# oneam/h264bsd

Hardware: AMD Instinct MI355X
Metric: 1080p macroblocks/s (higher is better)
Workload: dtype u8; 1 GPU; 256 concurrent copies of test_1920x1080.h264 per GPU (73 pictures x 8160 MB), kernel-only replay from HBM-resident frame jobs, inter+intra reconstruction + in-loop deblocking; streams_per_gpu=256, parallelism=streams/1, stream_groups=1, row_bands=library default (engine.hip TailConfig)

## Files before the change

### h264bsd_amd/capi.py

```python
import ctypes
import os
import subprocess

import numpy as np

HERE = os.path.dirname(os.path.abspath(__file__))
CSRC = os.path.join(HERE, "csrc")
LIB_PATH = os.path.join(HERE, "lib", "libh264bsd_mi355x.so")
BENCH_LIB_PATH = os.path.join(HERE, "lib", "libh264bsd_mi355x_bench.so")
if os.environ.get("H264BSD_VARIANT"):
    BENCH_LIB_PATH = os.path.join(HERE, "lib_" + os.environ["H264BSD_VARIANT"], "libh264bsd_mi355x_bench.so")

(H264BSD_RDY, H264BSD_PIC_RDY, H264BSD_HDRS_RDY, H264BSD_ERROR, H264BSD_PARAM_SET_ERROR,
 H264BSD_MEMALLOC_ERROR) = range(6)

EXPORTED_SYMBOLS = [
    "h264bsdInit", "h264bsdDecode", "h264bsdShutdown", "h264bsdNextOutputPicture",
    "h264bsdNextOutputPictureRGBA", "h264bsdNextOutputPictureBGRA", "h264bsdNextOutputPictureYCbCrA",
    "h264bsdPicWidth", "h264bsdPicHeight", "h264bsdVideoRange", "h264bsdMatrixCoefficients",
    "h264bsdCroppingParams", "h264bsdSampleAspectRatio", "h264bsdCheckValidParamSets", "h264bsdFlushBuffer",
    "h264bsdProfile", "h264bsdAlloc", "h264bsdFree", "h264bsdConvertToRGBA", "h264bsdConvertToBGRA",
    "h264bsdConvertToYCbCrA",
    "h264bsdmiInitCapture", "h264bsdmiNextOutputInfo", "h264bsdmiNextOutputPictureDevice", "h264bsdmiNextOutputTensorBatch", "h264bsdmiNextOutputTensorBatchColour", "h264bsdmiNextOutputTensorBatchResize", "h264bsdmiOutputTensorRegions", "h264bsdmiOutputTensorRemap", "h264bsdmiSetMotionExport", "h264bsdmiOutputMotionRegions", "h264bsdmiOutputRegionStats", "h264bsdmiKeepCurrentPictures", "h264bsdmiOutputRegionChange", "h264bsdmiOutputRegionShift", "h264bsdmiOutputCellMaps", "h264bsdmiOutputCellBoxes", "h264bsdmiJobFinalize", "h264bsdmiDeviceCount", "h264bsdmiSetDevice", "h264bsdmiFlush", "h264bsdmiFlushAsync", "h264bsdmiDeviceErrors",
    "h264bsdmiDecodePicture", "h264bsdmiDecodePictureBatch", "h264bsdmiNextOutputPictureBatch", "h264bsdmiPullAndDecodePictureBatch", "h264bsdmiSetParserThreads", "h264bsdmiSetInputReadOnly", "h264bsdmiSetCopyElision",
    "h264bsdmiReplayCreate", "h264bsdmiReplayCreateStaggered", "h264bsdmiReplayCreateDesync", "h264bsdmiReplayCreateSched", "h264bsdmiReplayReschedule", "h264bsdmiReplayDestroy", "h264bsdmiReplayRun", "h264bsdmiReplaySync",
    "h264bsdmiReplayFetch", "h264bsdmiReplayChecksums", "h264bsdmiReplayConvert", "h264bsdmiReplayFetchConverted",
    "h264bsdmiReplayTimings", "h264bsdmiReplaySetConvert", "h264bsdmiReplayConvertTimings", "h264bsdmiReplaySetStages", "h264bsdmiReplaySetTimedKernels", "h264bsdmiReplaySetGroups", "h264bsdmiDebugTailProfile", "h264bsdmiDebugSetTail", "h264bsdmiDebugDeviceErrorEvents", "h264bsdmiReplayJobBytes", "h264bsdmiReplayFrameBytes",
]

class DevicePicture(ctypes.Structure):
    _fields_ = [("data", ctypes.c_void_p), ("width", ctypes.c_uint32), ("height", ctypes.c_uint32), ("pitch", ctypes.c_uint32),
                ("format", ctypes.c_uint32), ("picId", ctypes.c_uint32), ("isIdrPic", ctypes.c_uint32),
                ("numErrMbs", ctypes.c_uint32), ("stream", ctypes.c_void_p)]


FMT_RGBA, FMT_BGRA, FMT_YCBCRA, FMT_I420 = 0, 1, 2, 3


class TensorSpec(ctypes.Structure):
    _fields_ = [("data", ctypes.c_void_p), ("width", ctypes.c_uint32), ("height", ctypes.c_uint32), ("layout", ctypes.c_uint32),
                ("dtype", ctypes.c_uint32), ("channels", ctypes.c_uint32), ("crop", ctypes.c_uint32), ("resize", ctypes.c_uint32),
                ("mean", ctypes.c_float * 3), ("std", ctypes.c_float * 3)]


class ColourSpec(ctypes.Structure):
    _fields_ = [("matrix", ctypes.c_uint32), ("range", ctypes.c_uint32), ("chroma", ctypes.c_uint32), ("unspecified", ctypes.c_uint32)]


class ResizeSpec(ctypes.Structure):
    _fields_ = [("filter", ctypes.c_uint32), ("fit", ctypes.c_uint32), ("pad", ctypes.c_float * 3)]


class Region(ctypes.Structure):
    _fields_ = [("instance", ctypes.c_uint32), ("x", ctypes.c_int), ("y", ctypes.c_int), ("w", ctypes.c_uint32), ("h", ctypes.c_uint32)]


class Remap(ctypes.Structure):
    _fields_ = [("instance", ctypes.c_uint32), ("map", ctypes.c_void_p)]

# ... 175 lines not shown
                                          P32, P32, P32, P32, P32]
    L.h264bsdmiOutputCellMaps.restype = ctypes.c_int
    L.h264bsdmiOutputCellBoxes.argtypes = [u32, ctypes.POINTER(vp), u32, ctypes.POINTER(Region), ctypes.POINTER(CellsSpec), ctypes.POINTER(BoxesSpec), vp,
                                           P32, P32, P32, P32, P32]
    L.h264bsdmiOutputCellBoxes.restype = ctypes.c_int
    L.h264bsdmiDecodePicture.argtypes = [vp, u8p, u32, u32, P32, P32]
    L.h264bsdmiDecodePicture.restype = u32
    L.h264bsdmiDecodePictureBatch.argtypes = [u32, ctypes.POINTER(vp), ctypes.POINTER(vp), P32, P32, P32, P32, P32]
    L.h264bsdmiPullAndDecodePictureBatch.argtypes = [u32, ctypes.POINTER(vp), ctypes.POINTER(vp), P32, P32, P32, ctypes.POINTER(vp), P32, P32, P32, P32, P32]
    L.h264bsdmiSetParserThreads.argtypes = [ctypes.c_int]
    L.h264bsdmiSetInputReadOnly.argtypes = [vp, u32]
    L.h264bsdmiSetCopyElision.argtypes = [vp, u32]
    L.h264bsdmiSetCopyElision.restype = ctypes.c_int
    L.h264bsdmiSetDevice.argtypes = [ctypes.c_int]
    L.h264bsdmiDeviceErrors.restype = ctypes.c_uint
    L.h264bsdmiNextOutputPictureBatch.argtypes = [u32, ctypes.POINTER(vp), ctypes.POINTER(vp), P32, P32, P32]
    if not harness:
        return L
    L.h264bsdmiJobFinalize.argtypes = [ctypes.c_void_p, u32, u32]
    L.h264bsdmiReplayCreate.argtypes = [ctypes.POINTER(ctypes.c_void_p), P32, u32, u32]
    L.h264bsdmiReplayCreate.restype = vp
    L.h264bsdmiReplayCreateStaggered.argtypes = [ctypes.POINTER(ctypes.c_void_p), P32, u32, u32, u32]
    L.h264bsdmiReplayCreateStaggered.restype = vp
    L.h264bsdmiReplayCreateDesync.argtypes = [ctypes.POINTER(ctypes.c_void_p), P32, u32, u32, P32, u32, u32]
    L.h264bsdmiReplayCreateDesync.restype = vp
    L.h264bsdmiReplayCreateSched.argtypes = [ctypes.POINTER(ctypes.c_void_p), P32, u32, u32, P32, u32, u32, u32]
    L.h264bsdmiReplayCreateSched.restype = vp
    L.h264bsdmiReplayReschedule.argtypes = [vp, P32, u32, u32, u32]
    L.h264bsdmiReplayDestroy.argtypes = [vp]
    L.h264bsdmiReplayDestroy.restype = None
    L.h264bsdmiReplayRun.argtypes = [vp, u32, u32]
    L.h264bsdmiReplaySync.argtypes = [vp]
    L.h264bsdmiReplayFetch.argtypes = [vp, u32, u32, vp]
    L.h264bsdmiReplayChecksums.argtypes = [vp, u32, vp]
    L.h264bsdmiReplayConvert.argtypes = [vp, u32, ctypes.c_int]
    L.h264bsdmiReplayFetchConverted.argtypes = [vp, u32, vp]
    L.h264bsdmiReplayTimings.argtypes = [vp, ctypes.POINTER(ctypes.c_float), P32]
    L.h264bsdmiReplaySetConvert.argtypes = [vp, ctypes.c_int]
    L.h264bsdmiReplayConvertTimings.argtypes = [vp, ctypes.POINTER(ctypes.c_float), P32]
    L.h264bsdmiReplaySetStages.argtypes = [vp, ctypes.c_uint]
    L.h264bsdmiReplaySetTimedKernels.argtypes = [vp, ctypes.c_uint]
    L.h264bsdmiReplaySetGroups.argtypes = [vp, u32]
    L.h264bsdmiDebugSetTail.argtypes = [u32] * 7
    L.h264bsdmiReplayJobBytes.argtypes = [vp]
    L.h264bsdmiReplayJobBytes.restype = ctypes.c_ulonglong
    L.h264bsdmiReplayFrameBytes.argtypes = [vp]
    L.h264bsdmiReplayFrameBytes.restype = u32
    return L


def device_count():
    return int(api_lib().h264bsdmiDeviceCount())


KEEP = 0xFFFFFFFF


def set_tail(dbk_rows_light=KEEP, dbk_rows_heavy=KEEP, dbk_waves=KEEP, intra_rows_light=KEEP, intra_rows_heavy=KEEP, intra_waves=KEEP,
             band_budget=KEEP):
    lib().h264bsdmiDebugSetTail(dbk_rows_light, dbk_rows_heavy, dbk_waves, intra_rows_light, intra_rows_heavy, intra_waves, band_budget)


def device_errors():
    return int(api_lib().h264bsdmiDeviceErrors())


# ... 798 lines not shown
        self.job_bytes = int(L.h264bsdmiReplayJobBytes(self._h))

    def reschedule(self, odd_offset=0, offsets=None, heavy_lanes=0, heavy_delay=4, groups=1):
        if offsets is None:
            offsets = [odd_offset if s & 1 else 0 for s in range(self.n_streams)]
        self.odd_offset = odd_offset
        self.offsets = [int(o) for o in offsets]
        offs = (ctypes.c_uint32 * self.n_streams)(*self.offsets)
        if self._L.h264bsdmiReplayReschedule(self._h, offs, heavy_lanes, heavy_delay, groups) != 0:
            raise RuntimeError("h264bsdmiReplayReschedule failed")

    def close(self):
        if self._h:
            self._L.h264bsdmiReplayDestroy(self._h)
            self._h = None

    __del__ = close

    def run(self, first=0, count=None):
        count = self.n_pics - first if count is None else count
        if self._L.h264bsdmiReplayRun(self._h, first, count) != 0:
            raise RuntimeError("h264bsdmiReplayRun failed")

    def sync(self):
        if self._L.h264bsdmiReplaySync(self._h) != 0:
            raise RuntimeError("h264bsdmiReplaySync failed")

    def fetch(self, stream, slot):
        out = np.empty(self.frame_bytes, dtype=np.uint8)
        if self._L.h264bsdmiReplayFetch(self._h, stream, slot, out.ctypes.data) != 0:
            raise RuntimeError("h264bsdmiReplayFetch failed")
        return out

    def checksums(self, slot):
        out = np.empty(self.n_streams, dtype=np.uint64)
        if self._L.h264bsdmiReplayChecksums(self._h, slot, out.ctypes.data) != 0:
            raise RuntimeError("h264bsdmiReplayChecksums failed")
        return out

    def set_convert(self, fmt, trailing=True, hosting=True, conv_waves=0):
        if fmt >= 0:
            fmt |= (0 if trailing else 0x100) | (0 if hosting else 0x200) | ((conv_waves & 15) << 16)
        if self._L.h264bsdmiReplaySetConvert(self._h, fmt) != 0:
            raise RuntimeError("h264bsdmiReplaySetConvert failed")

    def convert_timings(self):
        ms, n = ctypes.c_float(0), ctypes.c_uint32(0)
        if self._L.h264bsdmiReplayConvertTimings(self._h, ctypes.byref(ms), ctypes.byref(n)) != 0:
            raise RuntimeError("h264bsdmiReplayConvertTimings failed")
        return ms.value, n.value

    def convert(self, slot, fmt):
        if self._L.h264bsdmiReplayConvert(self._h, slot, fmt) != 0:
            raise RuntimeError("h264bsdmiReplayConvert failed")

    def fetch_converted(self, stream, n_pixels):
        out = np.empty(n_pixels, dtype=np.uint32)
        if self._L.h264bsdmiReplayFetchConverted(self._h, stream, out.ctypes.data) != 0:
            raise RuntimeError("h264bsdmiReplayFetchConverted failed")
        return out

    def set_groups(self, n):
        if self._L.h264bsdmiReplaySetGroups(self._h, n) != 0:
            raise RuntimeError('h264bsdmiReplaySetGroups failed')

    def set_stages(self, mask):
# ... 18 lines not shown
```

### h264bsd_amd/csrc/engine.hip

```cpp
#include <hip/hip_runtime.h>
#include <stdio.h>
#include <stdlib.h>
#include <string.h>
#include <deque>
#include <memory>
#include <mutex>
#include <vector>
#include <algorithm>
#include "kernels.hip.h"
#include "kernels/k_tensor_out.hip.h"
#include "kernels/k_tensor_aa.hip.h"
#include "kernels/k_tensor_roi.hip.h"
#include "kernels/k_tensor_remap.hip.h"
#include "kernels/k_motion.hip.h"
#include "kernels/k_region_stats.hip.h"
#include "kernels/k_keep.hip.h"
#include "kernels/k_region_change.hip.h"
#include "kernels/k_region_shift.hip.h"
#include "kernels/k_cell_maps.hip.h"
#include "kernels/k_cell_boxes.hip.h"
#include "engine.h"
#include "hip_owned.h"
#include "tick_plan.h"
#include "../../include/h264bsd_mi355x_bench.h"
// ... 301 lines not shown
        const bool heavy = h->n_intra * 4u > h->n_mbs;
        d.heavy = heavy ? 1 : 0;
        d.dbk_bands = bands_for(h->height_mbs, heavy ? tc.dbk_rows_heavy : tc.dbk_rows_light);
        d.intra_bands = h->intra_down_deps ? 1 : bands_for(h->height_mbs, heavy ? tc.intra_rows_heavy : tc.intra_rows_light);
    }
    d.err = dev_err;
    d.conv_src = nullptr; d.conv_dst = nullptr; d.conv_fmt = 0; d.conv_pad = 0;
    for (uint32_t k = 0; k < FJ_MAX_SLOTS; k++) d.slot[k] = k < h->n_slots ? dev_frames + (size_t)k * frame_bytes : nullptr;
    if (shape) {
        shape->n_frames++;
        shape->max_mbs = std::max(shape->max_mbs, h->n_mbs);
        shape->max_copy = std::max(shape->max_copy, h->n_copy);
        shape->max_gen = std::max(shape->max_gen, h->n_gen);
        shape->max_gen_uni = std::max(shape->max_gen_uni, h->n_gen_uniform);
        shape->max_gen_quad = std::max(shape->max_gen_quad, h->n_gen_quad);
        shape->max_gen_rest = std::max(shape->max_gen_rest, h->n_gen - h->n_gen_uniform - h->n_gen_quad);
        shape->max_dbk = std::max(shape->max_dbk, h->n_dbk);
        shape->any_deblock |= h->any_deblock != 0;
        shape->max_levels = std::max(shape->max_levels, h->n_intra_levels);
        shape->max_w = std::max<uint32_t>(shape->max_w, h->width_mbs);
        shape->max_h = std::max<uint32_t>(shape->max_h, h->height_mbs);
        shape->any_tail |= h->n_intra_levels != 0 || h->any_deblock != 0;
        shape->n_heavy += d.heavy;
        if (h->any_deblock) (d.heavy ? shape->want_heavy : shape->want_light)[0] = std::max<uint32_t>((d.heavy ? shape->want_heavy : shape->want_light)[0], d.dbk_bands);
        if (h->n_intra_levels) (d.heavy ? shape->want_heavy : shape->want_light)[1] = std::max<uint32_t>((d.heavy ? shape->want_heavy : shape->want_light)[1], d.intra_bands);
        if (h->n_intra_levels && h->intra_down_deps) shape->intra_whole = true;
    }
}

struct TickTimers { Event ev[6]; Event sev[5]; bool on = false; bool copy_timed = false; unsigned mask = 31u; };

static void launch_kdbk(hipStream_t st, const FrameDesc *d_desc, const TickShape &s, uint32_t launches[5])
{
    hipLaunchKernelGGL(h264k::k_dbk, dim3(std::min<uint32_t>((s.max_dbk + 4 * DBK_WG_WAVES - 1) / (4 * DBK_WG_WAVES), DBK_WGS * 4 / DBK_WG_WAVES), s.n_frames), dim3(64 * DBK_WG_WAVES), 0, st, d_desc);
    if (launches) launches[2]++;
}
template <int PATH> static void launch_inter(hipStream_t st, const FrameDesc *d_desc, uint32_t n_max, uint32_t n_frames)
{
    constexpr uint32_t per_wg = INTER_WG_WAVES * h264k::inter_per_wave<PATH>();
    if (n_max) hipLaunchKernelGGL(h264k::k_recon_inter<PATH>, dim3((n_max + per_wg - 1) / per_wg, n_frames), dim3(64 * INTER_WG_WAVES), 0, st, d_desc);
}
std::mutex g_tail_lds_mu;
size_t g_tail_lds[2][2][MAX_DEVICES] = {};
static int tail_prepare(hipStream_t st, int which, const BandPlan &bp, const void *fn, uint32_t **tickets)
{
    const bool banded = bp.bands > 1;
    *tickets = banded ? tickets_for(st) : nullptr;
    if (banded && !*tickets) return -1;
    int dev = 0;
    HIP_TRY(hipGetDevice(&dev));
    std::lock_guard<std::mutex> lk(g_tail_lds_mu);
    if (bp.lds > g_tail_lds[which][banded][dev]) {
        HIP_TRY(hipFuncSetAttribute(fn, hipFuncAttributeMaxDynamicSharedMemorySize, (int)bp.lds));
        g_tail_lds[which][banded][dev] = bp.lds;
    }
    return 0;
}

int launch_tick(hipStream_t st, const FrameDesc *d_desc, const TickShape &s, TickTimers *tt, uint32_t launches[5],
                unsigned stages = 7u, const SideLane *side = nullptr, unsigned long long *prof = nullptr)
{
    const bool timed = tt && tt->on;
    const unsigned tmask = timed ? tt->mask : 0u;
    auto boundary = [&](unsigned i) -> int {
        if ((((tmask << 1) | tmask) >> i) & 1u) HIP_TRY(hipEventRecord(tt->ev[i], st));
        return 0;
    };
// ... 1344 lines not shown
```

### h264bsd_amd/csrc/kernels/k_dbk.hip.h

```cpp
#pragma once
namespace h264k {
#ifndef DBK_WGS
#define DBK_WGS 32
#endif
#ifndef DBK_WG_WAVES
#define DBK_WG_WAVES 4
#endif
__global__ __launch_bounds__(64 * DBK_WG_WAVES) void k_dbk(const FrameDesc *__restrict__ frames)
{
    __shared__ uint32_t s_tab[32 + 64];
    if (threadIdx.x < 64) {
        const uint32_t t = threadIdx.x, ok = t < 52;
        reinterpret_cast<uint8_t *>(s_tab)[t] = ok ? c_alpha[t] : 0;
        reinterpret_cast<uint8_t *>(s_tab)[64 + t] = ok ? c_beta[t] : 0;
        s_tab[32 + t] = ok ? (uint32_t)c_tc0[t][0] | ((uint32_t)c_tc0[t][1] << 8) | ((uint32_t)c_tc0[t][2] << 16) : 0u;
    }
    __syncthreads();
    const FrameDesc &fd = FD_REF(frames, blockIdx.y);
    const int m = threadIdx.x & 15;
    const int wmb = fd.wmb;
    const uint32_t n_dbk = fd.n_dbk;
    uint32_t di = blockIdx.x * (4 * DBK_WG_WAVES) + (threadIdx.x >> 4);
    const bool live0 = di < n_dbk;
    if (__ballot(live0) == 0ull) return;
    uint32_t mb = live0 ? fd.dbki[di] : 0u;
    bool live = live0;
  for (;;) {
    const uint32_t ndi = di + (4u * DBK_WG_WAVES) * gridDim.x;
    uint32_t nmb = mb;
    const bool nlive = live && ndi < n_dbk;
    if (nlive) nmb = fd.dbki[ndi];
    const uint32_t mbx = mb - mb_row(fd, mb) * (uint32_t)wmb;
    const uint32_t mbl = mbx ? mb - 1 : mb, mbt = mb >= (uint32_t)wmb ? mb - wmb : mb;
    FjMbRec q, pl, pt;
    const int dir = m >> 3, e = (m >> 1) & 3, kh = m & 1;
    int qx[2], qy[2], px[2], py[2];
    uint32_t mva[2], mvb[2];
#pragma unroll
    for (int kk = 0; kk < 2; kk++) {
        const int k = 2 * kh + kk;
        qx[kk] = dir ? k : e; qy[kk] = dir ? e : k;
        px[kk] = dir ? k : (e ? e - 1 : 3); py[kk] = dir ? (e ? e - 1 : 3) : k;
    }
    {
        const H264K_GLOBAL uint8_t *rq = (const H264K_GLOBAL uint8_t *)(fd.recs + mb), *rl = (const H264K_GLOBAL uint8_t *)(fd.recs + mbl),
                                   *rt = (const H264K_GLOBAL uint8_t *)(fd.recs + mbt);
        uint4 w[6] = { ld16g(rq), ld16g(rq + 16), ld16g(rl), ld16g(rl + 16), ld16g(rt), ld16g(rt + 16) };
#pragma unroll
        for (int i = 0; i < 6; i++) asm volatile("" : "+v"(w[i].x), "+v"(w[i].y), "+v"(w[i].z), "+v"(w[i].w));
        __builtin_memcpy(&q, &w[0], 32); __builtin_memcpy(&pl, &w[2], 32); __builtin_memcpy(&pt, &w[4], 32);
    }
    {
        const FjMbRec &pr = e ? q : (dir ? pt : pl);
        const bool q_one = (q.pred & FJ_PRED_UNIFORM_MV) || q.kind != FJ_MB_INTER, p_one = (pr.pred & FJ_PRED_UNIFORM_MV) || pr.kind != FJ_MB_INTER;
        const uint32_t q_mv = q.kind == FJ_MB_INTER ? (uint32_t)(uint16_t)q.mv[0] | ((uint32_t)(uint16_t)q.mv[1] << 16) : 0u;
        const uint32_t p_mv = pr.kind == FJ_MB_INTER ? (uint32_t)(uint16_t)pr.mv[0] | ((uint32_t)(uint16_t)pr.mv[1] << 16) : 0u;
#pragma unroll
        for (int kk = 0; kk < 2; kk++) {
            mva[kk] = q_mv; mvb[kk] = p_mv;
            if (!q_one) mva[kk] = *(const H264K_GLOBAL uint32_t *)(fd.mvx + 32 * (size_t)q.mvx + 2 * (4 * qy[kk] + qx[kk]));
            if (!p_one) mvb[kk] = *(const H264K_GLOBAL uint32_t *)(fd.mvx + 32 * (size_t)pr.mvx + 2 * (4 * py[kk] + px[kk]));
        }
    }
    uint8_t *out = fd.dbk + (size_t)mb * DBK_REC_BYTES;
    uint8_t *any_out = fd.dbk + (size_t)fd.n_mbs * DBK_REC_BYTES + mb;
    const bool filtered = live && q.dbk && q.kind != FJ_MB_ABSENT;
    if (live && !filtered && m == 0) { *reinterpret_cast<uint16_t *>(out + 46) = 0; *any_out = 0; }
    uint32_t bs2 = 0;
    const bool f_left = (q.dbk & FJ_DBK_LEFT) && mbx, f_top = (q.dbk & FJ_DBK_TOP) && mb >= (uint32_t)wmb;
    if (filtered) {
        const bool edge_on = e ? true : (dir ? f_top : f_left);
        if (edge_on) {
            const int p_kind = e ? q.kind : (dir ? pt.kind : pl.kind);
            const int parts = (q.pred >> FJ_PRED_PARTS_SHIFT) & 3;
            const uint32_t p_coded = e ? q.coded : (dir ? pt.coded : pl.coded);
            uint32_t qrefs, prefs, t0, t1;
            __builtin_memcpy(&qrefs, q.ref_slot, 4);
            __builtin_memcpy(&t0, pl.ref_slot, 4);
            __builtin_memcpy(&t1, pt.ref_slot, 4);
            prefs = e ? qrefs : (dir ? t1 : t0);
            const bool intra_edge = is_intra_kind(q.kind) || is_intra_kind(p_kind);
            const bool no_motion_edge = e && (parts == FJ_PARTS_16x16 || (parts == FJ_PARTS_16x8 && !(dir == 1 && e == 2)) || (parts == FJ_PARTS_8x16 && !(dir == 0 && e == 2)));
#pragma unroll
            for (int kk = 0; kk < 2; kk++) {
                int my_bs;
                if (intra_edge) my_bs = e ? 3 : 4;
                else if (((q.coded >> z_of(qx[kk], qy[kk])) & 1) || ((p_coded >> z_of(px[kk], py[kk])) & 1)) my_bs = 2;
                else if (no_motion_edge) my_bs = 0;
                else if (((qrefs >> (8 * ((qy[kk] >> 1) * 2 + (qx[kk] >> 1)))) & 255u) != ((prefs >> (8 * ((py[kk] >> 1) * 2 + (px[kk] >> 1)))) & 255u)) my_bs = 1;
                else {
                    const int ax = (int16_t)(mva[kk] & 0xFFFFu), ay = (int32_t)mva[kk] >> 16, bx2 = (int16_t)(mvb[kk] & 0xFFFFu), by2 = (int32_t)mvb[kk] >> 16;
                    my_bs = (abs(ax - bx2) >= 4 || abs(ay - by2) >= 4) ? 1 : 0;
                }
                bs2 |= (uint32_t)my_bs << (4 * kk);
            }
        }
    }
    uint32_t v = bs2;
    v |= (uint32_t)__builtin_amdgcn_update_dpp(0, (int)v, 0x101, 0xF, 0xF, true) << 8;
    v |= (uint32_t)__builtin_amdgcn_update_dpp(0, (int)v, 0x102, 0xF, 0xF, true) << 16;
    const unsigned long long bal = __ballot(bs2 != 0u);
    const uint32_t bal16 = (uint32_t)(bal >> (threadIdx.x & 48)) & 0xFFFFu;
    const bool any = bal16 != 0u;
    const uint32_t sched = (any ? DBKF_ANY : 0u) | ((bal16 & 0x0003u) ? DBKF_LEFT : 0u) | ((bal16 & 0x0300u) ? DBKF_TOP : 0u) |
                           ((bal16 & 0xFCFCu) ? DBKF_INNER : 0u);
    if (filtered) {
        if ((m & 3) == 0) *reinterpret_cast<uint32_t *>(out + m) = v;
        if (m < 6) {
            const int c = m;
            const int side = c % 3;
            const int pqp = side == 0 ? (int)pl.qp_y : side == 1 ? (int)pt.qp_y : (int)q.qp_y;
            int a = (int)q.qp_y, b = pqp;
            if (c >= 3) {
                a = qpc_of(clip3(0, 51, a + q.cqp_off));
                b = qpc_of(clip3(0, 51, b + q.cqp_off));
            }
            const int qpav = (a + b + 1) >> 1;
            const int ia = clip3(0, 51, qpav + q.alpha_off), ib = clip3(0, 51, qpav + q.beta_off);
            const uint32_t t = s_tab[32 + ia];
            *reinterpret_cast<uint32_t *>(out + 16 + 4 * c) = (uint32_t)reinterpret_cast<const uint8_t *>(s_tab)[ia] |
                ((uint32_t)reinterpret_cast<const uint8_t *>(s_tab)[64 + ib] << 8) | ((t & 0xFFFFu) << 16);
            out[40 + c] = (uint8_t)(t >> 16);
        }
        if (m == 12) {
            *reinterpret_cast<uint16_t *>(out + 46) = (uint16_t)((f_left ? FJ_DBK_LEFT : 0u) | (f_top ? FJ_DBK_TOP : 0u) | (q.dbk & FJ_DBK_INNER) | (any ? 0x100u : 0u));
            *any_out = (uint8_t)sched;
        }
    }
    if (__ballot(nlive) == 0ull) return;
    di = ndi; mb = nmb; live = nlive;
  }
}

}
```

### h264bsd_amd/csrc/replay.hip.h

```cpp
extern "C" {
unsigned h264bsdmiDebugDeviceErrorEvents(void) { return poll_all_devices(true); }

#ifdef H264K_INTER_PROFILE
int h264bsdmiDebugReadCounters(unsigned long long *out)
{
    Engine *e = engine_get();
    if (!e) return -1;
    HIP_TRY(hipSetDevice(e->device));
    HIP_TRY(hipDeviceSynchronize());
    HIP_TRY(hipMemcpy(out, reinterpret_cast<uint8_t *>(e->d_err) + 64, 192, hipMemcpyDeviceToHost));
    HIP_TRY(hipMemset(reinterpret_cast<uint8_t *>(e->d_err) + 64, 0, 192));
    HIP_TRY(hipDeviceSynchronize());
    return 0;
}
#endif

struct h264bsdmi_replay {
    Engine *e;
    uint32_t n_pics, n_streams, n_slots, wmb, hmb, frame_bytes;
    size_t blob_stride;
    unsigned long long job_bytes;
    DeviceMem<uint8_t> d_blobs;
    DeviceMem<uint8_t> d_frames;
    DeviceMem<uint8_t> d_dbk;
// ... 416 lines not shown
                float ms;
                if (!((r->timed_mask >> k) & 1u)) continue;
                HIP_TRY(hipEventElapsedTime(&ms, r->timers[i].ev[k], r->timers[i].ev[k + 1]));
                out_ms[k] += ms;
            }
            if ((r->timed_mask & 4u) && r->overlap_dbk && !(r->stages & 8u) && r->n_groups == 1 && r->timers[i].sev[0] &&
                hipEventQuery(r->timers[i].sev[2]) == hipSuccess) {
                float ms;
                if (hipEventElapsedTime(&ms, r->timers[i].sev[1], r->timers[i].sev[2]) == hipSuccess) out_ms[2] += ms;
            }
            if (r->timers[i].copy_timed && hipEventQuery(r->timers[i].sev[4]) == hipSuccess) {
                float ms;
                if (hipEventElapsedTime(&ms, r->timers[i].sev[3], r->timers[i].sev[4]) == hipSuccess) out_ms[0] += ms;
            }
        }
    if (r->timed_count || !r->sched.empty()) HIP_TRY(hipEventElapsedTime(&out_ms[5], r->ev_begin, r->ev_end));
    if (launches) for (int k = 0; k < 5; k++) launches[k] = r->launches[k];
    return 0;
}

int h264bsdmiReplayFetch(h264bsdmi_replay *r, u32 stream, u32 slot, u8 *dst)
{
    if (!r || stream >= r->n_streams || slot >= r->n_slots) return -1;
    HIP_TRY(hipSetDevice(r->e->device));
    std::lock_guard<std::mutex> lk(r->e->mu);
    if (!r->d_planar) HIP_TRY(r->d_planar.alloc(r->frame_bytes));
    hipLaunchKernelGGL(h264k::k_detile, dim3(512, 1), dim3(256), 0, r->e->stream, r->d_frames + ((size_t)stream * r->n_slots + slot) * r->frame_bytes,
                       r->d_planar, r->wmb, r->hmb, (size_t)0, (size_t)0);
    HIP_TRY(hipMemcpyAsync(dst, r->d_planar, r->frame_bytes, hipMemcpyDeviceToHost, r->e->stream));
    HIP_TRY(hipStreamSynchronize(r->e->stream));
    return 0;
}

int h264bsdmiReplayChecksums(h264bsdmi_replay *r, u32 slot, unsigned long long *sums)
{
    if (!r || slot >= r->n_slots) return -1;
    std::lock_guard<std::mutex> lk(r->e->mu);
    HIP_TRY(hipSetDevice(r->e->device));
    hipLaunchKernelGGL(h264k::k_checksum, dim3(r->n_streams), dim3(256), 0, r->e->stream,
                       r->d_frames + (size_t)slot * r->frame_bytes, (size_t)r->n_slots * r->frame_bytes, r->wmb, r->hmb, r->d_sums);
    HIP_TRY(hipMemcpyAsync(sums, r->d_sums, sizeof(unsigned long long) * r->n_streams, hipMemcpyDeviceToHost, r->e->stream));
    if (poll_errors(r->e)) return -1;
    return 0;
}

int h264bsdmiReplayConvert(h264bsdmi_replay *r, u32 slot, int fmt)
{
    if (!r || slot >= r->n_slots || fmt < 0 || fmt > 2) return -1;
    std::lock_guard<std::mutex> lk(r->e->mu);
    HIP_TRY(hipSetDevice(r->e->device));
    const uint32_t w = r->wmb * 16, h = r->hmb * 16;
    if (!r->d_conv) HIP_TRY(r->d_conv.alloc((size_t)w * h * 4 * r->n_streams));
    hipLaunchKernelGGL(h264k::k_convert_tiles, CONVERT_GRID(r->n_streams), dim3(256), 0, r->e->stream,
                       r->d_frames + (size_t)slot * r->frame_bytes, r->d_conv, r->wmb, r->hmb, fmt,
                       (size_t)r->n_slots * r->frame_bytes, (size_t)w * h);
    HIP_TRY(hipGetLastError());
    return 0;
}

int h264bsdmiReplayFetchConverted(h264bsdmi_replay *r, u32 stream, u32 *dst)
{
    if (!r || stream >= r->n_streams || !r->d_conv) return -1;
    HIP_TRY(hipSetDevice(r->e->device));
    HIP_TRY(hipStreamSynchronize(r->e->stream));
    const size_t n = (size_t)r->wmb * 16 * r->hmb * 16;
    HIP_TRY(hipMemcpy(dst, r->d_conv + (size_t)stream * n, n * 4, hipMemcpyDeviceToHost));
// ... 103 lines not shown
```

### include/h264bsd_mi355x_bench.h

```cpp
#ifndef H264BSD_MI355X_BENCH_H
#define H264BSD_MI355X_BENCH_H

#include "h264bsd_mi355x.h"

#ifdef __cplusplus
extern "C" {
#endif

int h264bsdmiJobFinalize(u8 *job, u32 capacity, u32 n_coef_blocks);

typedef struct h264bsdmi_replay h264bsdmi_replay;
h264bsdmi_replay *h264bsdmiReplayCreate(const u8 *const *blobs, const u32 *bytes, u32 n_pics, u32 n_streams);
h264bsdmi_replay *h264bsdmiReplayCreateStaggered(const u8 *const *blobs, const u32 *bytes, u32 n_pics, u32 n_streams,
                                                 u32 odd_offset);
h264bsdmi_replay *h264bsdmiReplayCreateDesync(const u8 *const *blobs, const u32 *bytes, u32 n_pics, u32 n_streams,
                                              const u32 *offsets, u32 heavy_lanes, u32 heavy_delay);
h264bsdmi_replay *h264bsdmiReplayCreateSched(const u8 *const *blobs, const u32 *bytes, u32 n_pics, u32 n_streams,
                                             const u32 *offsets, u32 heavy_lanes, u32 heavy_delay, u32 groups);
int  h264bsdmiReplayReschedule(h264bsdmi_replay *r, const u32 *offsets, u32 heavy_lanes, u32 heavy_delay, u32 groups);
void h264bsdmiReplayDestroy(h264bsdmi_replay *r);
int  h264bsdmiReplayRun(h264bsdmi_replay *r, u32 first, u32 count);
int  h264bsdmiReplaySync(h264bsdmi_replay *r);
int  h264bsdmiReplayFetch(h264bsdmi_replay *r, u32 stream, u32 slot, u8 *dst);
int  h264bsdmiReplayChecksums(h264bsdmi_replay *r, u32 slot, unsigned long long *sums);
int  h264bsdmiReplayConvert(h264bsdmi_replay *r, u32 slot, int fmt);
int  h264bsdmiReplayFetchConverted(h264bsdmi_replay *r, u32 stream, u32 *dst);
int  h264bsdmiReplayTimings(h264bsdmi_replay *r, float out_ms[6], u32 launches[5]);
int  h264bsdmiReplaySetGroups(h264bsdmi_replay *r, u32 n_groups);
int  h264bsdmiReplaySetStages(h264bsdmi_replay *r, unsigned mask);
int  h264bsdmiReplaySetTimedKernels(h264bsdmi_replay *r, unsigned mask);
int  h264bsdmiReplaySetConvert(h264bsdmi_replay *r, int fmt);
int  h264bsdmiReplayConvertTimings(h264bsdmi_replay *r, float *ms, u32 *launches);
int  h264bsdmiDebugTailProfile(int enable, unsigned long long *out);
int  h264bsdmiDebugSetTail(u32 dbk_rows_light, u32 dbk_rows_heavy, u32 dbk_waves, u32 intra_rows_light, u32 intra_rows_heavy, u32 intra_waves,
                           u32 band_budget);
unsigned h264bsdmiDebugDeviceErrorEvents(void);
unsigned long long h264bsdmiReplayJobBytes(h264bsdmi_replay *r);
u32  h264bsdmiReplayFrameBytes(h264bsdmi_replay *r);
#ifdef __cplusplus
}
#endif
#endif
```

Measured before the change: 1.767 billion macroblocks/s.

## Compute deblock boundary strengths one macroblock per thread with bitwise packing

The deblock-strength kernel moves from 16 lanes per macroblock with a grid-stride persistent loop to one thread per macroblock. Boundary strengths for all edges are computed with packed bit manipulation (raster/transpose of coded masks, spread into nibbles), and motion vectors are loaded as 16-byte vectors. Each record is written with three 16-byte stores instead of scattered partial writes. A debug entry point is added to dump these records for validation. Per-thread register pressure and divergence rise, and the grid now scales with the macroblock count rather than being capped.

```diff
diff --git a/h264bsd_amd/capi.py b/h264bsd_amd/capi.py
--- a/h264bsd_amd/capi.py
+++ b/h264bsd_amd/capi.py
@@ -24,7 +24,7 @@
     "h264bsdmiInitCapture", "h264bsdmiNextOutputInfo", "h264bsdmiNextOutputPictureDevice", "h264bsdmiNextOutputTensorBatch", "h264bsdmiNextOutputTensorBatchColour", "h264bsdmiNextOutputTensorBatchResize", "h264bsdmiOutputTensorRegions", "h264bsdmiOutputTensorRemap", "h264bsdmiSetMotionExport", "h264bsdmiOutputMotionRegions", "h264bsdmiOutputRegionStats", "h264bsdmiKeepCurrentPictures", "h264bsdmiOutputRegionChange", "h264bsdmiOutputRegionShift", "h264bsdmiOutputCellMaps", "h264bsdmiOutputCellBoxes", "h264bsdmiJobFinalize", "h264bsdmiDeviceCount", "h264bsdmiSetDevice", "h264bsdmiFlush", "h264bsdmiFlushAsync", "h264bsdmiDeviceErrors",
     "h264bsdmiDecodePicture", "h264bsdmiDecodePictureBatch", "h264bsdmiNextOutputPictureBatch", "h264bsdmiPullAndDecodePictureBatch", "h264bsdmiSetParserThreads", "h264bsdmiSetInputReadOnly", "h264bsdmiSetCopyElision",
     "h264bsdmiReplayCreate", "h264bsdmiReplayCreateStaggered", "h264bsdmiReplayCreateDesync", "h264bsdmiReplayCreateSched", "h264bsdmiReplayReschedule", "h264bsdmiReplayDestroy", "h264bsdmiReplayRun", "h264bsdmiReplaySync",
-    "h264bsdmiReplayFetch", "h264bsdmiReplayChecksums", "h264bsdmiReplayConvert", "h264bsdmiReplayFetchConverted",
+    "h264bsdmiReplayFetch", "h264bsdmiReplayDbkRecords", "h264bsdmiReplayChecksums", "h264bsdmiReplayConvert", "h264bsdmiReplayFetchConverted",
     "h264bsdmiReplayTimings", "h264bsdmiReplaySetConvert", "h264bsdmiReplayConvertTimings", "h264bsdmiReplaySetStages", "h264bsdmiReplaySetTimedKernels", "h264bsdmiReplaySetGroups", "h264bsdmiDebugTailProfile", "h264bsdmiDebugSetTail", "h264bsdmiDebugDeviceErrorEvents", "h264bsdmiReplayJobBytes", "h264bsdmiReplayFrameBytes",
 ]
 
@@ -266,6 +266,7 @@
     L.h264bsdmiReplayRun.argtypes = [vp, u32, u32]
     L.h264bsdmiReplaySync.argtypes = [vp]
     L.h264bsdmiReplayFetch.argtypes = [vp, u32, u32, vp]
+    L.h264bsdmiReplayDbkRecords.argtypes = [vp, u32, u32, vp, u32]
     L.h264bsdmiReplayChecksums.argtypes = [vp, u32, vp]
     L.h264bsdmiReplayConvert.argtypes = [vp, u32, ctypes.c_int]
     L.h264bsdmiReplayFetchConverted.argtypes = [vp, u32, vp]
@@ -1130,6 +1131,13 @@
             raise RuntimeError("h264bsdmiReplayFetch failed")
         return out
 
+    def dbk_records(self, picture, stream):
+        n = self.frame_bytes // 384
+        out = np.empty(n * 48 + ((n + 3) & ~3), dtype=np.uint8)
+        if self._L.h264bsdmiReplayDbkRecords(self._h, picture, stream, out.ctypes.data, out.size) != 0:
+            raise RuntimeError("h264bsdmiReplayDbkRecords failed")
+        return out[:n * 48].reshape(n, 48), out[n * 48:n * 48 + n]
+
     def checksums(self, slot):
         out = np.empty(self.n_streams, dtype=np.uint64)
         if self._L.h264bsdmiReplayChecksums(self._h, slot, out.ctypes.data) != 0:
diff --git a/h264bsd_amd/csrc/engine.hip b/h264bsd_amd/csrc/engine.hip
--- a/h264bsd_amd/csrc/engine.hip
+++ b/h264bsd_amd/csrc/engine.hip
@@ -357,7 +357,7 @@
 
 static void launch_kdbk(hipStream_t st, const FrameDesc *d_desc, const TickShape &s, uint32_t launches[5])
 {
-    hipLaunchKernelGGL(h264k::k_dbk, dim3(std::min<uint32_t>((s.max_dbk + 4 * DBK_WG_WAVES - 1) / (4 * DBK_WG_WAVES), DBK_WGS * 4 / DBK_WG_WAVES), s.n_frames), dim3(64 * DBK_WG_WAVES), 0, st, d_desc);
+    hipLaunchKernelGGL(h264k::k_dbk, dim3((s.max_dbk + 64 * DBK_WG_WAVES - 1) / (64 * DBK_WG_WAVES), s.n_frames), dim3(64 * DBK_WG_WAVES), 0, st, d_desc);
     if (launches) launches[2]++;
 }
 template <int PATH> static void launch_inter(hipStream_t st, const FrameDesc *d_desc, uint32_t n_max, uint32_t n_frames)
diff --git a/h264bsd_amd/csrc/kernels/k_dbk.hip.h b/h264bsd_amd/csrc/kernels/k_dbk.hip.h
--- a/h264bsd_amd/csrc/kernels/k_dbk.hip.h
+++ b/h264bsd_amd/csrc/kernels/k_dbk.hip.h
@@ -1,135 +1,169 @@
 #pragma once
 namespace h264k {
-#ifndef DBK_WGS
-#define DBK_WGS 32
+#ifndef DBK_WG_WAVES
+#define DBK_WG_WAVES 8
 #endif
-#ifndef DBK_WG_WAVES
-#define DBK_WG_WAVES 4
-#endif
+
+__host__ __device__ __forceinline__ uint32_t dbk_raster16(uint32_t z) { return (z & 0xC3C3u) | ((z & 0x0C0Cu) << 2) | ((z & 0x3030u) >> 2); }
+__host__ __device__ __forceinline__ uint32_t dbk_transpose16(uint32_t r)
+{
+    uint32_t t = (r ^ (r >> 3)) & 0x0A0Au;
+    r ^= t ^ (t << 3);
+    t = (r ^ (r >> 6)) & 0x00CCu;
+    return r ^ t ^ (t << 6);
+}
+__host__ __device__ __forceinline__ uint32_t dbk_spread8(uint32_t b)
+{
+    b = (b | (b << 12)) & 0x000F000Fu;
+    b = (b | (b << 6)) & 0x03030303u;
+    return (b | (b << 3)) & 0x11111111u;
+}
+__host__ __device__ __forceinline__ bool dbk_mv_differ(uint32_t a, uint32_t b)
+{
+    const int dx = (int)(int16_t)(a & 0xFFFFu) - (int)(int16_t)(b & 0xFFFFu), dy = ((int32_t)a >> 16) - ((int32_t)b >> 16);
+    return (uint32_t)(dx + 3) > 6u || (uint32_t)(dy + 3) > 6u;
+}
+__host__ __device__ __forceinline__ bool dbk_ref_differ(uint32_t a, int i, uint32_t b, int j) { return ((a >> (8 * i)) & 255u) != ((b >> (8 * j)) & 255u); }
+__host__ __device__ __forceinline__ uint32_t dbk_ref_bits(int dir, uint32_t q, uint32_t p)
+{
+    return dir == 0 ? (dbk_ref_differ(q, 0, p, 1) ? 0x0003u : 0u) | (dbk_ref_differ(q, 2, p, 3) ? 0x000Cu : 0u) |
+                      (dbk_ref_differ(q, 1, q, 0) ? 0x0300u : 0u) | (dbk_ref_differ(q, 3, q, 2) ? 0x0C00u : 0u)
+                    : (dbk_ref_differ(q, 0, p, 2) ? 0x0003u : 0u) | (dbk_ref_differ(q, 1, p, 3) ? 0x000Cu : 0u) |
+                      (dbk_ref_differ(q, 2, q, 0) ? 0x0300u : 0u) | (dbk_ref_differ(q, 3, q, 1) ? 0x0C00u : 0u);
+}
+__host__ __device__ __forceinline__ uint32_t dbk_compared(int dir, int parts)
+{
+    return parts == FJ_PARTS_8x8 ? 0xFFFFu : parts == (dir ? FJ_PARTS_16x8 : FJ_PARTS_8x16) ? 0x0F0Fu : 0x000Fu;
+}
+__host__ __device__ __forceinline__ uint2 dbk_dir_strengths(uint32_t cq, uint32_t p_edge, bool q_intra, bool p_intra, uint32_t motion, bool edge_on)
+{
+    uint32_t lo = 0x33334444u, hi = 0x33333333u;
+    if (!q_intra) {
+        const uint32_t two = (cq | (cq << 4) | p_edge) & 0xFFFFu, one = motion & ~two;
+        lo = 2u * dbk_spread8(two & 255u) | dbk_spread8(one & 255u);
+        hi = 2u * dbk_spread8(two >> 8) | dbk_spread8((one >> 8) & 255u);
+        if (p_intra) lo = (lo & 0xFFFF0000u) | 0x4444u;
+    }
+    if (!edge_on) lo &= 0xFFFF0000u;
+    return make_uint2(lo, hi);
+}
+__host__ __device__ __forceinline__ uint2 dbk_mv_bits(const uint32_t mq[16], const uint32_t ml[4], const uint32_t mt[4])
+{
+    uint32_t d0 = 0, d1 = 0;
+#pragma unroll
+    for (int e = 0; e < 4; e++)
+#pragma unroll
+        for (int k = 0; k < 4; k++) {
+            if (dbk_mv_differ(mq[4 * k + e], e ? mq[4 * k + e - 1] : ml[k])) d0 |= 1u << (4 * e + k);
+            if (dbk_mv_differ(mq[4 * e + k], e ? mq[4 * (e - 1) + k] : mt[k])) d1 |= 1u << (4 * e + k);
+        }
+    return make_uint2(d0, d1);
+}
+
 __global__ __launch_bounds__(64 * DBK_WG_WAVES) void k_dbk(const FrameDesc *__restrict__ frames)
 {
     __shared__ uint32_t s_tab[32 + 64];
-    if (threadIdx.x < 64) {
-        const uint32_t t = threadIdx.x, ok = t < 52;
-        reinterpret_cast<uint8_t *>(s_tab)[t] = ok ? c_alpha[t] : 0;
-        reinterpret_cast<uint8_t *>(s_tab)[64 + t] = ok ? c_beta[t] : 0;
-        s_tab[32 + t] = ok ? (uint32_t)c_tc0[t][0] | ((uint32_t)c_tc0[t][1] << 8) | ((uint32_t)c_tc0[t][2] << 16) : 0u;
-    }
-    __syncthreads();
     const FrameDesc &fd = FD_REF(frames, blockIdx.y);
-    const int m = threadIdx.x & 15;
     const int wmb = fd.wmb;
     const uint32_t n_dbk = fd.n_dbk;
-    uint32_t di = blockIdx.x * (4 * DBK_WG_WAVES) + (threadIdx.x >> 4);
-    const bool live0 = di < n_dbk;
-    if (__ballot(live0) == 0ull) return;
-    uint32_t mb = live0 ? fd.dbki[di] : 0u;
-    bool live = live0;
-  for (;;) {
-    const uint32_t ndi = di + (4u * DBK_WG_WAVES) * gridDim.x;
-    uint32_t nmb = mb;
-    const bool nlive = live && ndi < n_dbk;
-    if (nlive) nmb = fd.dbki[ndi];
+    if (blockIdx.x * (64u * DBK_WG_WAVES) >= n_dbk) return;
+    const uint32_t di = blockIdx.x * (64u * DBK_WG_WAVES) + threadIdx.x;
+    const bool live = di < n_dbk;
+    const uint32_t mb = live ? fd.dbki[di] : 0u;
     const uint32_t mbx = mb - mb_row(fd, mb) * (uint32_t)wmb;
     const uint32_t mbl = mbx ? mb - 1 : mb, mbt = mb >= (uint32_t)wmb ? mb - wmb : mb;
     FjMbRec q, pl, pt;
-    const int dir = m >> 3, e = (m >> 1) & 3, kh = m & 1;
-    int qx[2], qy[2], px[2], py[2];
-    uint32_t mva[2], mvb[2];
-#pragma unroll
-    for (int kk = 0; kk < 2; kk++) {
-        const int k = 2 * kh + kk;
-        qx[kk] = dir ? k : e; qy[kk] = dir ? e : k;
-        px[kk] = dir ? k : (e ? e - 1 : 3); py[kk] = dir ? (e ? e - 1 : 3) : k;
-    }
     {
         const H264K_GLOBAL uint8_t *rq = (const H264K_GLOBAL uint8_t *)(fd.recs + mb), *rl = (const H264K_GLOBAL uint8_t *)(fd.recs + mbl),
                                    *rt = (const H264K_GLOBAL uint8_t *)(fd.recs + mbt);
         uint4 w[6] = { ld16g(rq), ld16g(rq + 16), ld16g(rl), ld16g(rl + 16), ld16g(rt), ld16g(rt + 16) };
+        if (threadIdx.x < 64) {
+            const uint32_t t = threadIdx.x, ok = t < 52;
+            reinterpret_cast<uint8_t *>(s_tab)[t] = ok ? c_alpha[t] : 0;
+            reinterpret_cast<uint8_t *>(s_tab)[64 + t] = ok ? c_beta[t] : 0;
+            s_tab[32 + t] = ok ? (uint32_t)c_tc0[t][0] | ((uint32_t)c_tc0[t][1] << 8) | ((uint32_t)c_tc0[t][2] << 16) : 0u;
+        }
+        __syncthreads();
 #pragma unroll
         for (int i = 0; i < 6; i++) asm volatile("" : "+v"(w[i].x), "+v"(w[i].y), "+v"(w[i].z), "+v"(w[i].w));
         __builtin_memcpy(&q, &w[0], 32); __builtin_memcpy(&pl, &w[2], 32); __builtin_memcpy(&pt, &w[4], 32);
     }
-    {
-        const FjMbRec &pr = e ? q : (dir ? pt : pl);
-        const bool q_one = (q.pred & FJ_PRED_UNIFORM_MV) || q.kind != FJ_MB_INTER, p_one = (pr.pred & FJ_PRED_UNIFORM_MV) || pr.kind != FJ_MB_INTER;
-        const uint32_t q_mv = q.kind == FJ_MB_INTER ? (uint32_t)(uint16_t)q.mv[0] | ((uint32_t)(uint16_t)q.mv[1] << 16) : 0u;
-        const uint32_t p_mv = pr.kind == FJ_MB_INTER ? (uint32_t)(uint16_t)pr.mv[0] | ((uint32_t)(uint16_t)pr.mv[1] << 16) : 0u;
-#pragma unroll
-        for (int kk = 0; kk < 2; kk++) {
-            mva[kk] = q_mv; mvb[kk] = p_mv;
-            if (!q_one) mva[kk] = *(const H264K_GLOBAL uint32_t *)(fd.mvx + 32 * (size_t)q.mvx + 2 * (4 * qy[kk] + qx[kk]));
-            if (!p_one) mvb[kk] = *(const H264K_GLOBAL uint32_t *)(fd.mvx + 32 * (size_t)pr.mvx + 2 * (4 * py[kk] + px[kk]));
-        }
-    }
+    if (__ballot(live) == 0ull) return;
     uint8_t *out = fd.dbk + (size_t)mb * DBK_REC_BYTES;
     uint8_t *any_out = fd.dbk + (size_t)fd.n_mbs * DBK_REC_BYTES + mb;
     const bool filtered = live && q.dbk && q.kind != FJ_MB_ABSENT;
-    if (live && !filtered && m == 0) { *reinterpret_cast<uint16_t *>(out + 46) = 0; *any_out = 0; }
-    uint32_t bs2 = 0;
+    if (live && !filtered) { *reinterpret_cast<uint16_t *>(out + 46) = 0; *any_out = 0; }
     const bool f_left = (q.dbk & FJ_DBK_LEFT) && mbx, f_top = (q.dbk & FJ_DBK_TOP) && mb >= (uint32_t)wmb;
-    if (filtered) {
-        const bool edge_on = e ? true : (dir ? f_top : f_left);
-        if (edge_on) {
-            const int p_kind = e ? q.kind : (dir ? pt.kind : pl.kind);
-            const int parts = (q.pred >> FJ_PRED_PARTS_SHIFT) & 3;
-            const uint32_t p_coded = e ? q.coded : (dir ? pt.coded : pl.coded);
-            uint32_t qrefs, prefs, t0, t1;
-            __builtin_memcpy(&qrefs, q.ref_slot, 4);
-            __builtin_memcpy(&t0, pl.ref_slot, 4);
-            __builtin_memcpy(&t1, pt.ref_slot, 4);
-            prefs = e ? qrefs : (dir ? t1 : t0);
-            const bool intra_edge = is_intra_kind(q.kind) || is_intra_kind(p_kind);
-            const bool no_motion_edge = e && (parts == FJ_PARTS_16x16 || (parts == FJ_PARTS_16x8 && !(dir == 1 && e == 2)) || (parts == FJ_PARTS_8x16 && !(dir == 0 && e == 2)));
+    const bool q_intra = is_intra_kind(q.kind), l_intra = is_intra_kind(pl.kind), t_intra = is_intra_kind(pt.kind);
+    const bool q_inter = q.kind == FJ_MB_INTER, l_inter = pl.kind == FJ_MB_INTER, t_inter = pt.kind == FJ_MB_INTER;
+    const uint32_t q_mv = q_inter ? (uint32_t)(uint16_t)q.mv[0] | ((uint32_t)(uint16_t)q.mv[1] << 16) : 0u;
+    const uint32_t l_mv = l_inter ? (uint32_t)(uint16_t)pl.mv[0] | ((uint32_t)(uint16_t)pl.mv[1] << 16) : 0u;
+    const uint32_t t_mv = t_inter ? (uint32_t)(uint16_t)pt.mv[0] | ((uint32_t)(uint16_t)pt.mv[1] << 16) : 0u;
+    const bool compares = filtered && q_inter;
+    const bool q_many = compares && !(q.pred & FJ_PRED_UNIFORM_MV);
+    const bool l_many = compares && f_left && l_inter && !(pl.pred & FJ_PRED_UNIFORM_MV);
+    const bool t_many = compares && f_top && t_inter && !(pt.pred & FJ_PRED_UNIFORM_MV);
+    uint2 mvd = make_uint2(dbk_mv_differ(q_mv, l_mv) ? 0x000Fu : 0u, dbk_mv_differ(q_mv, t_mv) ? 0x000Fu : 0u);
+    if (__ballot(q_many || l_many || t_many) != 0ull) {
+        if (q_many || l_many || t_many) {
+            uint32_t mq[16], ml[4], mt[4];
 #pragma unroll
-            for (int kk = 0; kk < 2; kk++) {
-                int my_bs;
-                if (intra_edge) my_bs = e ? 3 : 4;
-                else if (((q.coded >> z_of(qx[kk], qy[kk])) & 1) || ((p_coded >> z_of(px[kk], py[kk])) & 1)) my_bs = 2;
-                else if (no_motion_edge) my_bs = 0;
-                else if (((qrefs >> (8 * ((qy[kk] >> 1) * 2 + (qx[kk] >> 1)))) & 255u) != ((prefs >> (8 * ((py[kk] >> 1) * 2 + (px[kk] >> 1)))) & 255u)) my_bs = 1;
-                else {
-                    const int ax = (int16_t)(mva[kk] & 0xFFFFu), ay = (int32_t)mva[kk] >> 16, bx2 = (int16_t)(mvb[kk] & 0xFFFFu), by2 = (int32_t)mvb[kk] >> 16;
-                    my_bs = (abs(ax - bx2) >= 4 || abs(ay - by2) >= 4) ? 1 : 0;
-                }
-                bs2 |= (uint32_t)my_bs << (4 * kk);
+            for (int i = 0; i < 16; i++) mq[i] = q_mv;
+#pragma unroll
+            for (int i = 0; i < 4; i++) { ml[i] = l_mv; mt[i] = t_mv; }
+            if (q_many) {
+                const H264K_GLOBAL uint8_t *v = (const H264K_GLOBAL uint8_t *)(fd.mvx + 32 * (size_t)q.mvx);
+#pragma unroll
+                for (int i = 0; i < 4; i++) { const uint4 r = ld16g(v + 16 * i); mq[4 * i] = r.x; mq[4 * i + 1] = r.y; mq[4 * i + 2] = r.z; mq[4 * i + 3] = r.w; }
             }
+            if (l_many) {
+                const H264K_GLOBAL uint32_t *v = (const H264K_GLOBAL uint32_t *)(fd.mvx + 32 * (size_t)pl.mvx);
+#pragma unroll
+                for (int i = 0; i < 4; i++) ml[i] = v[4 * i + 3];
+            }
+            if (t_many) {
+                const uint4 r = ld16g((const H264K_GLOBAL uint8_t *)(fd.mvx + 32 * (size_t)pt.mvx) + 48);
+                mt[0] = r.x; mt[1] = r.y; mt[2] = r.z; mt[3] = r.w;
+            }
+            mvd = dbk_mv_bits(mq, ml, mt);
         }
     }
-    uint32_t v = bs2;
-    v |= (uint32_t)__builtin_amdgcn_update_dpp(0, (int)v, 0x101, 0xF, 0xF, true) << 8;
-    v |= (uint32_t)__builtin_amdgcn_update_dpp(0, (int)v, 0x102, 0xF, 0xF, true) << 16;
-    const unsigned long long bal = __ballot(bs2 != 0u);
-    const uint32_t bal16 = (uint32_t)(bal >> (threadIdx.x & 48)) & 0xFFFFu;
-    const bool any = bal16 != 0u;
-    const uint32_t sched = (any ? DBKF_ANY : 0u) | ((bal16 & 0x0003u) ? DBKF_LEFT : 0u) | ((bal16 & 0x0300u) ? DBKF_TOP : 0u) |
-                           ((bal16 & 0xFCFCu) ? DBKF_INNER : 0u);
-    if (filtered) {
-        if ((m & 3) == 0) *reinterpret_cast<uint32_t *>(out + m) = v;
-        if (m < 6) {
-            const int c = m;
-            const int side = c % 3;
-            const int pqp = side == 0 ? (int)pl.qp_y : side == 1 ? (int)pt.qp_y : (int)q.qp_y;
-            int a = (int)q.qp_y, b = pqp;
-            if (c >= 3) {
-                a = qpc_of(clip3(0, 51, a + q.cqp_off));
-                b = qpc_of(clip3(0, 51, b + q.cqp_off));
-            }
-            const int qpav = (a + b + 1) >> 1;
-            const int ia = clip3(0, 51, qpav + q.alpha_off), ib = clip3(0, 51, qpav + q.beta_off);
-            const uint32_t t = s_tab[32 + ia];
-            *reinterpret_cast<uint32_t *>(out + 16 + 4 * c) = (uint32_t)reinterpret_cast<const uint8_t *>(s_tab)[ia] |
-                ((uint32_t)reinterpret_cast<const uint8_t *>(s_tab)[64 + ib] << 8) | ((t & 0xFFFFu) << 16);
-            out[40 + c] = (uint8_t)(t >> 16);
+    if (!filtered) return;
+    uint32_t qrefs, lrefs, trefs;
+    __builtin_memcpy(&qrefs, q.ref_slot, 4);
+    __builtin_memcpy(&lrefs, pl.ref_slot, 4);
+    __builtin_memcpy(&trefs, pt.ref_slot, 4);
+    const int parts = (q.pred >> FJ_PRED_PARTS_SHIFT) & 3;
+    const uint32_t cq1 = dbk_raster16(q.coded & 0xFFFFu), cq0 = dbk_transpose16(cq1);
+    const uint32_t lc = pl.coded, tc = pt.coded;
+    const uint32_t l_edge = ((lc >> 5) & 1u) | ((lc >> 6) & 2u) | ((lc >> 11) & 4u) | ((lc >> 12) & 8u);
+    const uint32_t t_edge = ((tc >> 10) & 3u) | ((tc >> 12) & 12u);
+    const uint2 s0 = dbk_dir_strengths(cq0, l_edge, q_intra, l_intra, (dbk_ref_bits(0, qrefs, lrefs) | mvd.x) & dbk_compared(0, parts), f_left);
+    const uint2 s1 = dbk_dir_strengths(cq1, t_edge, q_intra, t_intra, (dbk_ref_bits(1, qrefs, trefs) | mvd.y) & dbk_compared(1, parts), f_top);
+    const uint32_t left = s0.x & 0xFFFFu, top = s1.x & 0xFFFFu, inner = (s0.x >> 16) | s0.y | (s1.x >> 16) | s1.y;
+    const bool any = (left | top | inner) != 0u;
+    const uint32_t sched = (any ? DBKF_ANY : 0u) | (left ? DBKF_LEFT : 0u) | (top ? DBKF_TOP : 0u) | (inner ? DBKF_INNER : 0u);
+    uint32_t thr[6], tc3[6];
+#pragma unroll
+    for (int c = 0; c < 6; c++) {
+        const int side = c % 3;
+        int a = (int)q.qp_y, b = side == 0 ? (int)pl.qp_y : side == 1 ? (int)pt.qp_y : (int)q.qp_y;
+        if (c >= 3) {
+            a = qpc_of(clip3(0, 51, a + q.cqp_off));
+            b = qpc_of(clip3(0, 51, b + q.cqp_off));
         }
-        if (m == 12) {
-            *reinterpret_cast<uint16_t *>(out + 46) = (uint16_t)((f_left ? FJ_DBK_LEFT : 0u) | (f_top ? FJ_DBK_TOP : 0u) | (q.dbk & FJ_DBK_INNER) | (any ? 0x100u : 0u));
-            *any_out = (uint8_t)sched;
-        }
+        const int qpav = (a + b + 1) >> 1;
+        const int ia = clip3(0, 51, qpav + q.alpha_off), ib = clip3(0, 51, qpav + q.beta_off);
+        const uint32_t t = s_tab[32 + ia];
+        thr[c] = (uint32_t)reinterpret_cast<const uint8_t *>(s_tab)[ia] | ((uint32_t)reinterpret_cast<const uint8_t *>(s_tab)[64 + ib] << 8) | ((t & 0xFFFFu) << 16);
+        tc3[c] = (t >> 16) & 255u;
     }
-    if (__ballot(nlive) == 0ull) return;
-    di = ndi; mb = nmb; live = nlive;
-  }
+    const uint32_t tail = (f_left ? FJ_DBK_LEFT : 0u) | (f_top ? FJ_DBK_TOP : 0u) | (q.dbk & FJ_DBK_INNER) | (any ? 0x100u : 0u);
+    H264K_GLOBAL uint8_t *o = (H264K_GLOBAL uint8_t *)out;
+    st16g(o, make_uint4(s0.x, s0.y, s1.x, s1.y));
+    st16g(o + 16, make_uint4(thr[0], thr[1], thr[2], thr[3]));
+    st16g(o + 32, make_uint4(thr[4], thr[5], tc3[0] | (tc3[1] << 8) | (tc3[2] << 16) | (tc3[3] << 24), tc3[4] | (tc3[5] << 8) | (tail << 16)));
+    *any_out = (uint8_t)sched;
 }
 
 }
diff --git a/h264bsd_amd/csrc/replay.hip.h b/h264bsd_amd/csrc/replay.hip.h
--- a/h264bsd_amd/csrc/replay.hip.h
+++ b/h264bsd_amd/csrc/replay.hip.h
@@ -472,6 +472,27 @@
     return 0;
 }
 
+int h264bsdmiReplayDbkRecords(h264bsdmi_replay *r, u32 picture, u32 stream, u8 *dst, u32 bytes)
+{
+    if (!r || picture >= r->n_pics || stream >= r->n_streams || !r->sched.empty() || r->n_groups > 1) return -1;
+    const size_t n_mbs = (size_t)r->wmb * r->hmb, n4 = (n_mbs + 3u) & ~(size_t)3u;
+    if (!dst || bytes != n_mbs * DBK_REC_BYTES + n4) return -1;
+    Engine *e = r->e;
+    std::lock_guard<std::mutex> lk(e->mu);
+    HIP_TRY(hipSetDevice(e->device));
+    HIP_TRY(hipStreamSynchronize(e->stream));
+    const TickShape &s = r->shapes[picture];
+    if (s.any_deblock && s.max_dbk) {
+        launch_kdbk(e->stream, r->d_desc + (size_t)picture * r->n_streams, s, nullptr);
+        HIP_TRY(hipGetLastError());
+    }
+    HIP_TRY(hipMemcpyAsync(dst, r->d_dbk + (size_t)stream * r->dbk_stride, bytes, hipMemcpyDeviceToHost, e->stream));
+    for (u32 k = 0; k < r->n_streams; k++)
+        HIP_TRY(hipMemsetAsync(r->d_dbk + (size_t)k * r->dbk_stride + n_mbs * DBK_REC_BYTES, 0, n4, e->stream));
+    HIP_TRY(hipStreamSynchronize(e->stream));
+    return 0;
+}
+
 int h264bsdmiReplayChecksums(h264bsdmi_replay *r, u32 slot, unsigned long long *sums)
 {
     if (!r || slot >= r->n_slots) return -1;
diff --git a/include/h264bsd_mi355x_bench.h b/include/h264bsd_mi355x_bench.h
--- a/include/h264bsd_mi355x_bench.h
+++ b/include/h264bsd_mi355x_bench.h
@@ -22,6 +22,7 @@
 int  h264bsdmiReplayRun(h264bsdmi_replay *r, u32 first, u32 count);
 int  h264bsdmiReplaySync(h264bsdmi_replay *r);
 int  h264bsdmiReplayFetch(h264bsdmi_replay *r, u32 stream, u32 slot, u8 *dst);
+int  h264bsdmiReplayDbkRecords(h264bsdmi_replay *r, u32 picture, u32 stream, u8 *dst, u32 bytes);
 int  h264bsdmiReplayChecksums(h264bsdmi_replay *r, u32 slot, unsigned long long *sums);
 int  h264bsdmiReplayConvert(h264bsdmi_replay *r, u32 slot, int fmt);
 int  h264bsdmiReplayFetchConverted(h264bsdmi_replay *r, u32 stream, u32 *dst);
```

New measurement: 1.833 billion macroblocks/s, median of 6. 3.7% higher.
